# Zhongxu-Wang/ArtSpeech

Hardware: NVIDIA B200
Metric: synthesized_audio_seconds_per_second (higher is better)
Workload: dtype bf16 (vocoder) / f16 (acoustic) operands, f32 accumulate

## Files before the change

### artspeech_b200/csrc/conv_igemm_impl.cuh

```cuda
#pragma once
#include "tc_util.cuh"

namespace asb {

constexpr int CV_THREADS = 320;
constexpr int CV_MAX_TAPS = 32;

struct ConvArgs {
  int B, To, Fo, Cout, CoutP;
  int tT, tF, n_ttiles, n_ftiles;
  int ntaps, kchunks, stages;
  int tap_dt[CV_MAX_TAPS];
  int tap_df[CV_MAX_TAPS];
  uint32_t idesc;
  const float* bias;
  const void* res1; int res1_dtype; long long res1_ld;
  const void* res2; int res2_dtype; long long res2_ld;
  float out_scale;
  void* y_raw; int y_raw_dtype; long long y_raw_ld; int y_raw_vec;
  void* y_act; int y_act_dtype; long long y_act_ld; int y_act_vec;
  int act; float slope;
  const int* lens;
  float* stats;
  int fast, k_res1, k_res2, k_raw, k_act, act_simple;
  float act_slope_eff;
  int halo_rows, pad_lo;
  int epi_tma;
  int halo_baseoff;
  int skip;
  int pad_stages;
};

struct EpiMaps { CUtensorMap r1, raw, act; };
__host__ __device__ constexpr uint32_t epi_cols(int bn) { return bn >= 64 ? 64u : 32u; }
__host__ __device__ constexpr uint32_t epi_warp_bytes(int bn) { return 2u * 32u * epi_cols(bn) * 2u; }
__host__ __device__ constexpr uint32_t epi_bytes(int bn) { return 8u * epi_warp_bytes(bn) + 64u; }


__device__ __forceinline__ bool conv_mtile_dead(const ConvArgs& a, int mt) {
  const int m = mt / a.n_ftiles;
  const int tt = m % a.n_ttiles, b = m / a.n_ttiles;
  if (b >= a.B) return true;
  return tt * a.tT >= __ldg(a.lens + b);
}
__device__ __forceinline__ bool conv_unit_skip(const ConvArgs& a, int unit, int cl) {
  if (!a.skip) return false;
  for (int r = 0; r < cl; ++r)
    if (!conv_mtile_dead(a, unit * cl + r)) return false;
  return true;
}
__device__ __forceinline__ void conv_zero_row(void* base, int dtype, long long off_elems, int ncols) {
  const int es = dtype == AS_F32 ? 4 : 2;
  char* p = reinterpret_cast<char*>(base) + off_elems * es;
  const int nbytes = ncols * es;
  int i = 0;
  if ((reinterpret_cast<uintptr_t>(p) & 15) == 0)
    for (; i + 16 <= nbytes; i += 16) *reinterpret_cast<uint4*>(p + i) = make_uint4(0u, 0u, 0u, 0u);
  for (; i < nbytes; i += es) {
    if (es == 4) *reinterpret_cast<float*>(p + i) = 0.f;
    else *reinterpret_cast<uint16_t*>(p + i) = 0;
  }
}
__device__ __forceinline__ void conv_zero_tile_row(const ConvArgs& a, int mt, int n0, int bn, int m) {
  const int it_ = m / a.tF, if_ = m - it_ * a.tF;
  int u = mt;
  const int ft = u % a.n_ftiles; u /= a.n_ftiles;
  const int tt = u % a.n_ttiles; u /= a.n_ttiles;
  const int b = u, t = tt * a.tT + it_, f = ft * a.tF + if_;
  if (b >= a.B || t >= a.To || f >= a.Fo) return;
  const int ncols = min(bn, a.Cout - n0);
  if (ncols <= 0) return;
  const long long row = ((long long)b * a.To + t) * a.Fo + f;
  if (a.y_raw != nullptr) conv_zero_row(a.y_raw, a.y_raw_dtype, row * a.y_raw_ld + n0, ncols);
  if (a.y_act != nullptr) conv_zero_row(a.y_act, a.y_act_dtype, row * a.y_act_ld + n0, ncols);
}

__device__ __forceinline__ void store16(void* base, int dtype, long long off, const float (&v)[16],
                                        int nvalid, bool vec) {
  if (dtype == AS_F32) {
    float* p = reinterpret_cast<float*>(base) + off;
    if (vec && nvalid == 16) {
      float4* p4 = reinterpret_cast<float4*>(p);
#pragma unroll
// ... 37 lines not shown
    if (vec && nvalid == 16) {
      const uint4* p4 = reinterpret_cast<const uint4*>(p);
#pragma unroll
      for (int h = 0; h < 2; ++h) {
        uint4 t = __ldg(p4 + h);
        uint32_t w[4] = {t.x, t.y, t.z, t.w};
#pragma unroll
        for (int i = 0; i < 4; ++i) {
          v[8 * h + 2 * i] += from16(uint16_t(w[i] & 0xFFFF), dtype);
          v[8 * h + 2 * i + 1] += from16(uint16_t(w[i] >> 16), dtype);
        }
      }
    } else {
#pragma unroll
      for (int i = 0; i < 16; ++i) if (i < nvalid) v[i] += from16(p[i], dtype);
    }
  }
}


template <bool BF16>
__device__ __forceinline__ void add_res_fast(const char* p, int kind, float (&v)[16]) {
  if (kind == 1) {
    const uint4 t0 = __ldg(reinterpret_cast<const uint4*>(p)), t1 = __ldg(reinterpret_cast<const uint4*>(p) + 1);
    unpack_add<BF16>(t0.x, v[0], v[1]); unpack_add<BF16>(t0.y, v[2], v[3]);
    unpack_add<BF16>(t0.z, v[4], v[5]); unpack_add<BF16>(t0.w, v[6], v[7]);
    unpack_add<BF16>(t1.x, v[8], v[9]); unpack_add<BF16>(t1.y, v[10], v[11]);
    unpack_add<BF16>(t1.z, v[12], v[13]); unpack_add<BF16>(t1.w, v[14], v[15]);
  } else {
#pragma unroll
    for (int i = 0; i < 4; ++i) {
      const float4 t = __ldg(reinterpret_cast<const float4*>(p) + i);
      v[4 * i] += t.x; v[4 * i + 1] += t.y; v[4 * i + 2] += t.z; v[4 * i + 3] += t.w;
    }
  }
}
template <bool BF16>
__device__ __forceinline__ void store_fast(char* p, int kind, const float (&v)[16]) {
  if (kind == 1) {
    uint4* q = reinterpret_cast<uint4*>(p);
    q[0] = make_uint4(pack2<BF16>(v[0], v[1]), pack2<BF16>(v[2], v[3]), pack2<BF16>(v[4], v[5]), pack2<BF16>(v[6], v[7]));
    q[1] = make_uint4(pack2<BF16>(v[8], v[9]), pack2<BF16>(v[10], v[11]), pack2<BF16>(v[12], v[13]), pack2<BF16>(v[14], v[15]));
  } else {
    float4* q = reinterpret_cast<float4*>(p);
#pragma unroll
    for (int i = 0; i < 4; ++i) q[i] = make_float4(v[4 * i], v[4 * i + 1], v[4 * i + 2], v[4 * i + 3]);
  }
}

template <int BN, bool BF16>
__device__ __forceinline__ void run_epilogue(const ConvArgs& a, uint32_t tmem_base, uint32_t tfull0,
                                             uint32_t tempty0, int warp, int lane, int m_tiles,
                                             int total_tiles, const float* bias_s, int tile_first = -1,
                                             int tile_step = 0, int cl = 1, int rank = 0, bool remote_tempty = false) {
  if (tile_first < 0) { tile_first = blockIdx.x; tile_step = gridDim.x; }
  constexpr int NPRE = (BN >= 256 ? 128 : (BN < 64 ? BN : 64)) / 8;
  auto tfull_bar = [&](int i) { return tfull0 + 8u * i; };
  auto tempty_bar = [&](int i) { return tempty0 + 8u * i; };
    const int wg = (warp - 2) >> 2;
  const int q = warp & 3;
  const int m = q * 32 + lane;
  const int it_ = m / a.tF, if_ = m - it_ * a.tF;
  int lt_live = 0;
  for (int tile = tile_first; tile < total_tiles; tile += tile_step) {
    if (conv_unit_skip(a, tile % m_tiles, cl)) {
      if (wg == 0) conv_zero_tile_row(a, (tile % m_tiles) * cl + rank, (tile / m_tiles) * BN, BN, m);
      continue;
    }
    const int lt = lt_live++;
    if ((lt & 1) != wg) continue;
    int mt = (tile % m_tiles) * cl + rank;
    const int n0 = (tile / m_tiles) * BN;
    const int ft = mt % a.n_ftiles; mt /= a.n_ftiles;
    const int tt = mt % a.n_ttiles; mt /= a.n_ttiles;
    const int b = mt;
    const int t = tt * a.tT + it_, f = ft * a.tF + if_;
    const bool row_ok = (t < a.To) && (f < a.Fo) && (b < a.B);
    bool masked = false;
    if (a.lens != nullptr && row_ok) masked = t >= __ldg(a.lens + b);
    const long long row = ((long long)b * a.To + t) * a.Fo + f;

    const int ncols = min(BN, a.Cout - n0);
    const bool fast = a.fast != 0;
    const int k_r1 = a.k_res1, k_r2 = a.k_res2, k_raw = a.k_raw, k_act = a.k_act;
    const char* p_r1 = k_r1 ? reinterpret_cast<const char*>(a.res1) + (row * a.res1_ld + n0) * (k_r1 == 1 ? 2 : 4) : nullptr;
    const char* p_r2 = k_r2 ? reinterpret_cast<const char*>(a.res2) + (row * a.res2_ld + n0) * (k_r2 == 1 ? 2 : 4) : nullptr;
    char* p_raw = k_raw ? reinterpret_cast<char*>(a.y_raw) + (row * a.y_raw_ld + n0) * (k_raw == 1 ? 2 : 4) : nullptr;
    char* p_act = k_act ? reinterpret_cast<char*>(a.y_act) + (row * a.y_act_ld + n0) * (k_act == 1 ? 2 : 4) : nullptr;
    const float scale = masked ? 0.f : a.out_scale;
    const float aslope = a.act_slope_eff;
    const float* bias_t = bias_s + n0;
    const bool pre_ok = fast && k_r1 == 1 && row_ok && !masked;
    uint4 pre[NPRE];
    if (pre_ok) {
#pragma unroll
      for (int i = 0; i < NPRE; ++i)
        if (i * 8 + 8 <= ncols) pre[i] = __ldg(reinterpret_cast<const uint4*>(p_r1) + i);
    }

    mbar_wait(tfull_bar(wg), ((uint32_t)lt >> 1) & 1u);
    tc_fence_after();
    const uint32_t tacc = tmem_base + (uint32_t)(wg * BN) + (uint32_t(q * 32) << 16);
#pragma unroll
    for (int cc = 0; cc < BN / 16; ++cc) {
      const int c0 = cc * 16;
      if (c0 >= ncols) break;
      uint32_t r[16];
      tc_ld16(tacc + uint32_t(c0), r);
      tc_wait_ld();
      if (!row_ok) continue;
      const int co = n0 + c0;
      float v[16];
#pragma unroll
      for (int i = 0; i < 16; ++i) v[i] = __uint_as_float(r[i]);
      if (fast && c0 + 16 <= ncols) {
        {
#pragma unroll
// ... 5 lines not shown
        if (pre_ok && 2 * cc + 1 < NPRE) {
          const uint4 t0 = pre[(2 * cc) < NPRE ? 2 * cc : 0], t1 = pre[(2 * cc + 1) < NPRE ? 2 * cc + 1 : 0];
          unpack_add<BF16>(t0.x, v[0], v[1]); unpack_add<BF16>(t0.y, v[2], v[3]);
          unpack_add<BF16>(t0.z, v[4], v[5]); unpack_add<BF16>(t0.w, v[6], v[7]);
          unpack_add<BF16>(t1.x, v[8], v[9]); unpack_add<BF16>(t1.y, v[10], v[11]);
          unpack_add<BF16>(t1.z, v[12], v[13]); unpack_add<BF16>(t1.w, v[14], v[15]);
        } else if (k_r1 && !masked) add_res_fast<BF16>(p_r1 + c0 * (k_r1 == 1 ? 2 : 4), k_r1, v);
        if (k_r2 && !masked) add_res_fast<BF16>(p_r2 + c0 * (k_r2 == 1 ? 2 : 4), k_r2, v);
#pragma unroll
        for (int i = 0; i < 16; ++i) v[i] *= scale;
        if (k_raw) store_fast<BF16>(p_raw + c0 * (k_raw == 1 ? 2 : 4), k_raw, v);
        if (k_act) {
          if (a.act_simple) {
#pragma unroll
            for (int i = 0; i < 16; ++i) v[i] = fmaxf(v[i], v[i] * aslope);
          } else {
#pragma unroll
            for (int i = 0; i < 16; ++i) v[i] = apply_act(v[i], a.act, a.slope);
          }
          store_fast<BF16>(p_act + c0 * (k_act == 1 ? 2 : 4), k_act, v);
        }
      } else {
        const int nvalid = min(16, a.Cout - co);
        if (a.bias != nullptr) {
#pragma unroll
          for (int i = 0; i < 16; ++i) if (i < nvalid) v[i] += __ldg(a.bias + co + i);
        }
        if (a.res1 != nullptr) add_res16(a.res1, a.res1_dtype, row * a.res1_ld + co, v, nvalid, false);
        if (a.res2 != nullptr) add_res16(a.res2, a.res2_dtype, row * a.res2_ld + co, v, nvalid, false);
#pragma unroll
        for (int i = 0; i < 16; ++i) v[i] = masked ? 0.f : v[i] * a.out_scale;
        if (a.y_raw != nullptr) store16(a.y_raw, a.y_raw_dtype, row * a.y_raw_ld + co, v, nvalid, false);
        if (a.y_act != nullptr) {
#pragma unroll
          for (int i = 0; i < 16; ++i) v[i] = apply_act(v[i], a.act, a.slope);
          store16(a.y_act, a.y_act_dtype, row * a.y_act_ld + co, v, nvalid, false);
        }
      }
    }
    tc_fence_before();
    __syncwarp();
    if (lane == 0) {
      if (remote_tempty) asm volatile("mbarrier.arrive.release.cluster.shared::cluster.b64 _, [%0];" ::"r"(tempty_bar(wg)) : "memory");
      else asm volatile("mbarrier.arrive.shared::cta.b64 _, [%0];" ::"r"(tempty_bar(wg)) : "memory");
    }
  }
}

template <int BN, bool BF16, bool F32 = false>
__device__ __forceinline__ void run_epilogue_tma(const ConvArgs& a, const EpiMaps& maps, uint32_t tmem_base,
                                                 uint32_t tfull0, uint32_t tempty0, int warp, int lane, int m_tiles,
                                                 int total_tiles, const float* bias_s, uint32_t epi_base,
                                                 int tile_first = -1, int tile_step = 0, int cl = 1, int rank = 0,
                                                 bool remote_tempty = false) {
  if (tile_first < 0) { tile_first = blockIdx.x; tile_step = gridDim.x; }
  const int ew = warp - 2;
  const int wg = ew >> 2;
  const int q = warp & 3;
  constexpr uint32_t EPC = F32 ? 32u : epi_cols(BN);
  constexpr uint32_t ROWA = F32 ? 128u : EPC * 2u;
  constexpr uint32_t ROWB = EPC * 2u;
  constexpr uint32_t TILEA = 32u * ROWA;
  constexpr int CPG = EPC / 16;
  const uint32_t bufA = epi_base + (uint32_t)ew * epi_warp_bytes(BN);
  const uint32_t bufB = bufA + epi_warp_bytes(BN) / 2u;
  const uint32_t rbar = epi_base + 8u * epi_warp_bytes(BN) + 8u * ew;
  const bool has_r1 = a.k_res1 != 0, has_raw = a.k_raw != 0, has_act = a.k_act != 0;
  const uint32_t rowoffA = (uint32_t)lane * ROWA, rowoffB = (uint32_t)lane * ROWB;
  const uint32_t swA = (ROWA == 128) ? (uint32_t)(lane & 7) : (uint32_t)((lane >> 1) & 3);
  const uint32_t swB = (ROWB == 128) ? (uint32_t)(lane & 7) : (uint32_t)((lane >> 1) & 3);
  uint32_t rphase = 0;
  int lt_live = 0;
  for (int tile = tile_first; tile < total_tiles; tile += tile_step) {
    if (conv_unit_skip(a, tile % m_tiles, cl)) {
      if (wg == 0) conv_zero_tile_row(a, (tile % m_tiles) * cl + rank, (tile / m_tiles) * BN, BN, q * 32 + lane);
      continue;
    }
    const int lt = lt_live++;
    if ((lt & 1) != wg) continue;
    const int mt = (tile % m_tiles) * cl + rank;
    const int n0 = (tile / m_tiles) * BN;
    const int tt = mt % a.n_ttiles, b = mt / a.n_ttiles;
    const int t_base = tt * 128 + q * 32;
    const int t = t_base + lane;
    const bool masked = (a.lens != nullptr) && (b < a.B) && (t < a.To) && (t >= __ldg(a.lens + b));
    const int ncols = min(BN, a.Cout - n0);
    const int ngroups = (ncols + (int)EPC - 1) / (int)EPC;
    const float scale = a.out_scale, aslope = a.act_slope_eff;

    if (has_r1 && lane == 0 && ngroups > 0) {
      bulk_wait_read0();
      mbar_expect_tx(rbar, TILEA);
      tma_load_3d(bufA, &maps.r1, rbar, n0, t_base, b);
    }
    mbar_wait(tfull0 + 8u * wg, ((uint32_t)lt >> 1) & 1u);
    tc_fence_after();
    const uint32_t tacc = tmem_base + (uint32_t)(wg * BN) + (uint32_t(q * 32) << 16);
    for (int g = 0; g < ngroups; ++g) {
      if (has_r1) {
        mbar_wait(rbar, rphase);
        rphase ^= 1u;
      } else {
        if (lane == 0) bulk_wait_read0();
        __syncwarp();
      }
#pragma unroll
      for (int cc = 0; cc < CPG; ++cc) {
        const int c0 = g * (int)EPC + cc * 16;
        if (c0 < ncols) {
          uint32_t r[16];
          tc_ld16(tacc + uint32_t(c0), r);
          tc_wait_ld();
          float v[16];
          const float* bt = bias_s + n0 + c0;
#pragma unroll
          for (int i = 0; i < 4; ++i) {
            const float4 bb = *reinterpret_cast<const float4*>(bt + 4 * i);
            v[4 * i] = __uint_as_float(r[4 * i]) + bb.x; v[4 * i + 1] = __uint_as_float(r[4 * i + 1]) + bb.y;
            v[4 * i + 2] = __uint_as_float(r[4 * i + 2]) + bb.z; v[4 * i + 3] = __uint_as_float(r[4 * i + 3]) + bb.w;
          }
          if constexpr (F32) {
            uint32_t oa[4];
#pragma unroll
            for (int j = 0; j < 4; ++j) oa[j] = bufA + rowoffA + (((uint32_t)(4 * cc + j) ^ swA) << 4);
            if (has_r1) {
#pragma unroll
// ... 37 lines not shown
            }
            const uint32_t b0 = bufB + rowoffB + (((uint32_t)(2 * cc) ^ swB) << 4), b1 = bufB + rowoffB + (((uint32_t)(2 * cc + 1) ^ swB) << 4);
            sts128(b0, make_uint4(pack2<BF16>(v[0], v[1]), pack2<BF16>(v[2], v[3]), pack2<BF16>(v[4], v[5]), pack2<BF16>(v[6], v[7])));
            sts128(b1, make_uint4(pack2<BF16>(v[8], v[9]), pack2<BF16>(v[10], v[11]), pack2<BF16>(v[12], v[13]), pack2<BF16>(v[14], v[15])));
          }
        }
      }
      fence_async_smem();
      __syncwarp();
      if (lane == 0) {
        if (has_raw) tma_store_3d(&maps.raw, bufA, n0 + g * (int)EPC, t_base, b);
        if (has_act) tma_store_3d(&maps.act, bufB, n0 + g * (int)EPC, t_base, b);
        bulk_commit();
        if (has_r1 && g + 1 < ngroups) {
          bulk_wait_read0();
          mbar_expect_tx(rbar, TILEA);
          tma_load_3d(bufA, &maps.r1, rbar, n0 + (g + 1) * (int)EPC, t_base, b);
        }
      }
      __syncwarp();
    }
    tc_fence_before();
    __syncwarp();
    if (lane == 0) {
      if (remote_tempty) asm volatile("mbarrier.arrive.release.cluster.shared::cluster.b64 _, [%0];" ::"r"(tempty0 + 8u * wg) : "memory");
      else asm volatile("mbarrier.arrive.shared::cta.b64 _, [%0];" ::"r"(tempty0 + 8u * wg) : "memory");
    }
  }
  if (lane == 0) bulk_wait_all0();
}

template <int BN, int BK, bool BF16>
__global__ void __launch_bounds__(CV_THREADS, (BN >= 256 ? 1 : 2))
conv_igemm_kernel(const __grid_constant__ CUtensorMap tmA, const __grid_constant__ CUtensorMap tmW,
                  const __grid_constant__ EpiMaps emaps,
                  const __grid_constant__ ConvArgs a) {
  constexpr int A_BYTES = 128 * BK * 2;
  constexpr int W_BYTES = BN * BK * 2;
  constexpr int STAGE_BYTES = A_BYTES + W_BYTES;
  constexpr int TMEM_COLS = (2 * BN) < 32 ? 32 : (2 * BN);

  extern __shared__ unsigned char smem_dyn[];
  const uint32_t smem_base = (smem_u32(smem_dyn) + 1023u) & ~1023u;
  const int S = a.stages;
  const uint32_t bar_base = smem_base + S * STAGE_BYTES;
  auto full_bar = [&](int s) { return bar_base + 8u * s; };
  auto empty_bar = [&](int s) { return bar_base + 8u * (S + s); };
  auto tfull_bar = [&](int i) { return bar_base + 8u * (2 * S + i); };
  auto tempty_bar = [&](int i) { return bar_base + 8u * (2 * S + 2 + i); };
  const uint32_t tmem_slot = bar_base + 8u * (2 * S + 4);
  float* bias_s = reinterpret_cast<float*>(smem_dyn + (bar_base + 8u * (2 * S + 6) - smem_u32(smem_dyn)));
  for (int i = threadIdx.x; i < a.CoutP; i += blockDim.x) bias_s[i] = (a.bias != nullptr && i < a.Cout) ? a.bias[i] : 0.f;
  const uint32_t epi_base = (bar_base + 8u * (2 * S + 6) + (uint32_t)a.CoutP * 4u + 1023u) & ~1023u;

  const int warp = threadIdx.x >> 5;
  const int lane = threadIdx.x & 31;
  const int m_tiles = a.B * a.n_ttiles * a.n_ftiles;
  const int total_tiles = m_tiles * (a.CoutP / BN);
  const int k_iters = a.ntaps * a.kchunks;

  if (threadIdx.x == 0) {
    for (int s = 0; s < S; ++s) { mbar_init(full_bar(s), 1); mbar_init(empty_bar(s), 1); }
    for (int i = 0; i < 2; ++i) { mbar_init(tfull_bar(i), 1); mbar_init(tempty_bar(i), 4); }
    if (a.epi_tma) for (int i = 0; i < 8; ++i) mbar_init(epi_base + 8u * epi_warp_bytes(BN) + 8u * i, 1);
    asm volatile("fence.mbarrier_init.release.cluster;" ::: "memory");
  }
  if (warp == 0 && lane == 0) {
    asm volatile("prefetch.tensormap [%0];" ::"l"(&tmA) : "memory");
    asm volatile("prefetch.tensormap [%0];" ::"l"(&tmW) : "memory");
  }
  if (warp == 1) {
    asm volatile("tcgen05.alloc.cta_group::1.sync.aligned.shared::cta.b32 [%0], %1;" ::"r"(tmem_slot),
                 "n"(TMEM_COLS)
                 : "memory");
    asm volatile("tcgen05.relinquish_alloc_permit.cta_group::1.sync.aligned;" ::: "memory");
  }
  tc_fence_before();
  __syncthreads();
  tc_fence_after();
  pdl_wait();
  uint32_t tmem_base;
  asm volatile("ld.shared.b32 %0, [%1];" : "=r"(tmem_base) : "r"(tmem_slot) : "memory");

  if (warp == 0) {
    if (lane == 0) {
      int it = 0;
      for (int tile = blockIdx.x; tile < total_tiles; tile += gridDim.x) {
        if (conv_unit_skip(a, tile % m_tiles, 1)) continue;
        int mt = tile % m_tiles;
        const int n0 = (tile / m_tiles) * BN;
        const int ft = mt % a.n_ftiles; mt /= a.n_ftiles;
        const int tt = mt % a.n_ttiles; mt /= a.n_ttiles;
        const int b = mt, t0 = tt * a.tT, f0 = ft * a.tF;
        for (int kit = 0; kit < k_iters; ++kit, ++it) {
          const int s = it % S;
          const uint32_t ph = (it / S) & 1;
          mbar_wait(empty_bar(s), ph ^ 1u);
          mbar_expect_tx(full_bar(s), STAGE_BYTES);
          const int tap = kit / a.kchunks, kc = kit - tap * a.kchunks;
          const uint32_t sa = smem_base + s * STAGE_BYTES;
          tma_load_4d(sa, &tmA, full_bar(s), kc * BK, f0 + a.tap_df[tap], t0 + a.tap_dt[tap], b);
          tma_load_2d(sa + A_BYTES, &tmW, full_bar(s), kc * BK, tap * a.CoutP + n0);
        }
      }
    }
  } else if (warp == 1) {
    if (elect_one()) {
      int it = 0, lt = 0;
      for (int tile = blockIdx.x; tile < total_tiles; tile += gridDim.x) {
        if (conv_unit_skip(a, tile % m_tiles, 1)) continue;
        const int acc = lt & 1;
        mbar_wait(tempty_bar(acc), (((uint32_t)lt >> 1) & 1u) ^ 1u);
        tc_fence_after();
        const uint32_t tacc = tmem_base + (uint32_t)(acc * BN);
        for (int kit = 0; kit < k_iters; ++kit, ++it) {
          const int s = it % S;
          const uint32_t ph = (it / S) & 1;
          mbar_wait(full_bar(s), ph);
          tc_fence_after();
          const uint32_t sa = smem_base + s * STAGE_BYTES;
          const uint64_t da = make_smem_desc<BK>(sa);
          const uint64_t db = make_smem_desc<BK>(sa + A_BYTES);
#pragma unroll
          for (int k = 0; k < BK / 16; ++k) {
            tc_mma_f16(tacc, da + uint64_t(2 * k), db + uint64_t(2 * k), a.idesc, (kit | k) != 0 ? 1u : 0u);
          }
          tc_commit(empty_bar(s));
        }
        tc_commit(tfull_bar(acc));
        ++lt;
      }
    }
  } else {
    if (a.epi_tma == 2) {
      if constexpr (BN >= 128)
        run_epilogue_tma<BN, BF16, true>(a, emaps, tmem_base, tfull_bar(0), tempty_bar(0), warp, lane, m_tiles, total_tiles, bias_s, epi_base);
    } else if (a.epi_tma)
      run_epilogue_tma<BN, BF16>(a, emaps, tmem_base, tfull_bar(0), tempty_bar(0), warp, lane, m_tiles, total_tiles, bias_s, epi_base);
    else
      run_epilogue<BN, BF16>(a, tmem_base, tfull_bar(0), tempty_bar(0), warp, lane, m_tiles, total_tiles, bias_s);
  }

  tc_fence_before();
  __syncthreads();
  if (warp == 1) {
    tc_fence_after();
    asm volatile("tcgen05.dealloc.cta_group::1.sync.aligned.b32 %0, %1;" ::"r"(tmem_base),
                 "n"(TMEM_COLS)
                 : "memory");
  }
}


template <int BK, bool BF16>
__global__ void __cluster_dims__(2, 1, 1) __launch_bounds__(CV_THREADS, 1)
conv_igemm_2cta_kernel(const __grid_constant__ CUtensorMap tmA, const __grid_constant__ CUtensorMap tmWh,
                       const __grid_constant__ EpiMaps emaps, const __grid_constant__ ConvArgs a) {
  constexpr int BN = 256;
  constexpr int A_BYTES = 128 * BK * 2;
  constexpr int WH_BYTES = (BN / 2) * BK * 2;
  constexpr int STAGE_BYTES = A_BYTES + WH_BYTES;
  constexpr int TMEM_COLS = 512;

  extern __shared__ unsigned char smem_dyn[];
  const uint32_t smem_base = ((smem_u32(smem_dyn) + 1023u) & ~1023u) + (uint32_t)a.pad_stages * STAGE_BYTES;
  const int S = a.stages;
  const uint32_t bar_base = smem_base + S * STAGE_BYTES;
  auto full_bar = [&](int s) { return bar_base + 8u * s; };
  auto empty_bar = [&](int s) { return bar_base + 8u * (S + s); };
  auto tfull_bar = [&](int i) { return bar_base + 8u * (2 * S + i); };
  auto tempty_bar = [&](int i) { return bar_base + 8u * (2 * S + 2 + i); };
  const uint32_t tmem_slot = bar_base + 8u * (2 * S + 4);
  float* bias_s = reinterpret_cast<float*>(smem_dyn + (bar_base + 8u * (2 * S + 6) - smem_u32(smem_dyn)));
  for (int i = threadIdx.x; i < a.CoutP; i += blockDim.x) bias_s[i] = (a.bias != nullptr && i < a.Cout) ? a.bias[i] : 0.f;
  const uint32_t epi_base = (bar_base + 8u * (2 * S + 6) + (uint32_t)a.CoutP * 4u + 1023u) & ~1023u;

  const int warp = threadIdx.x >> 5;
  const int lane = threadIdx.x & 31;
  const uint32_t rank = cluster_ctarank();
  const bool leader = rank == 0;
  const int m_tiles = a.B * a.n_ttiles * a.n_ftiles;
  const int m_pairs = (m_tiles + 1) / 2;
  const int total_super = m_pairs * (a.CoutP / BN);
  const int cid = blockIdx.x >> 1, n_clusters = gridDim.x >> 1;
  const int k_iters = a.ntaps * a.kchunks;

  if (threadIdx.x == 0) {
    for (int s = 0; s < S; ++s) { mbar_init(full_bar(s), 1); mbar_init(empty_bar(s), 1); }
    for (int i = 0; i < 2; ++i) { mbar_init(tfull_bar(i), 1); mbar_init(tempty_bar(i), 8); }
    if (a.epi_tma) for (int i = 0; i < 8; ++i) mbar_init(epi_base + 8u * epi_warp_bytes(BN) + 8u * i, 1);
    asm volatile("fence.mbarrier_init.release.cluster;" ::: "memory");
  }
  if (warp == 0 && lane == 0) {
    asm volatile("prefetch.tensormap [%0];" ::"l"(&tmA) : "memory");
    asm volatile("prefetch.tensormap [%0];" ::"l"(&tmWh) : "memory");
  }
  if (warp == 1) {
    asm volatile("tcgen05.alloc.cta_group::2.sync.aligned.shared::cta.b32 [%0], %1;" ::"r"(tmem_slot), "n"(TMEM_COLS) : "memory");
    asm volatile("tcgen05.relinquish_alloc_permit.cta_group::2.sync.aligned;" ::: "memory");
  }
  tc_fence_before();
  cluster_sync();
  tc_fence_after();
  pdl_wait();
  uint32_t tmem_base;
  asm volatile("ld.shared.b32 %0, [%1];" : "=r"(tmem_base) : "r"(tmem_slot) : "memory");

  if (warp == 0) {
    if (lane == 0) {
      int it = 0;
      for (int st = cid; st < total_super; st += n_clusters) {
        if (conv_unit_skip(a, st % m_pairs, 2)) continue;
        int mt = (st % m_pairs) * 2 + (int)rank;
        const int n0 = (st / m_pairs) * BN;
        const int ft = mt % a.n_ftiles; mt /= a.n_ftiles;
        const int tt = mt % a.n_ttiles; mt /= a.n_ttiles;
        const int b = mt, t0 = tt * a.tT, f0 = ft * a.tF;
        for (int kit = 0; kit < k_iters; ++kit, ++it) {
          const int s = it % S;
          const uint32_t ph = (it / S) & 1;
          mbar_wait(empty_bar(s), ph ^ 1u);
          if (leader) mbar_expect_tx(full_bar(s), 2u * STAGE_BYTES);
          const uint32_t fb = mapa_u32(full_bar(s), 0);
          const int tap = kit / a.kchunks, kc = kit - tap * a.kchunks;
          const uint32_t sa = smem_base + s * STAGE_BYTES;
          tma2_load_4d(sa, &tmA, fb, kc * BK, f0 + a.tap_df[tap], t0 + a.tap_dt[tap], b);
          tma2_load_2d(sa + A_BYTES, &tmWh, fb, kc * BK, tap * a.CoutP + n0 + (int)rank * (BN / 2));
        }
      }
    }
  } else if (warp == 1) {
    if (leader && elect_one()) {
      int it = 0, lt = 0;
      for (int st = cid; st < total_super; st += n_clusters) {
        if (conv_unit_skip(a, st % m_pairs, 2)) continue;
        const int acc = lt & 1;
        mbar_wait(tempty_bar(acc), (((uint32_t)lt >> 1) & 1u) ^ 1u);
        tc_fence_after();
        const uint32_t tacc = tmem_base + (uint32_t)(acc * BN);
        for (int kit = 0; kit < k_iters; ++kit, ++it) {
          const int s = it % S;
          const uint32_t ph = (it / S) & 1;
          mbar_wait(full_bar(s), ph);
          tc_fence_after();
          const uint32_t sa = smem_base + s * STAGE_BYTES;
          const uint64_t da = make_smem_desc<BK>(sa);
          const uint64_t db = make_smem_desc<BK>(sa + A_BYTES);
#pragma unroll
          for (int k = 0; k < BK / 16; ++k)
            tc2_mma_f16(tacc, da + uint64_t(2 * k), db + uint64_t(2 * k), a.idesc, (kit | k) != 0 ? 1u : 0u);
          tc2_commit(empty_bar(s));
        }
        tc2_commit(tfull_bar(acc));
        ++lt;
      }
    }
    __syncwarp();
  } else {
    const uint32_t tempty_leader = mapa_u32(tempty_bar(0), 0);
    if (a.epi_tma == 2)
      run_epilogue_tma<BN, BF16, true>(a, emaps, tmem_base, tfull_bar(0), tempty_leader, warp, lane, m_pairs, total_super, bias_s,
                                       epi_base, cid, n_clusters, 2, (int)rank, true);
    else if (a.epi_tma)
      run_epilogue_tma<BN, BF16>(a, emaps, tmem_base, tfull_bar(0), tempty_leader, warp, lane, m_pairs, total_super, bias_s, epi_base,
                                 cid, n_clusters, 2, (int)rank, true);
    else
      run_epilogue<BN, BF16>(a, tmem_base, tfull_bar(0), tempty_leader, warp, lane, m_pairs, total_super, bias_s,
                             cid, n_clusters, 2, (int)rank, true);
  }

  tc_fence_before();
  cluster_sync();
  if (warp == 1) {
    tc_fence_after();
    asm volatile("tcgen05.dealloc.cta_group::2.sync.aligned.b32 %0, %1;" ::"r"(tmem_base), "n"(TMEM_COLS) : "memory");
  }
}

__device__ __forceinline__ uint64_t make_desc_noswz(uint32_t saddr, uint32_t lbo_bytes) {
  return uint64_t((saddr >> 4) & 0x3FFF) | (uint64_t((lbo_bytes >> 4) & 0x3FFF) << 16) |
         (uint64_t(128 >> 4) << 32) | (uint64_t(1) << 46);
}

template <int BN, bool BF16>
__global__ void __launch_bounds__(CV_THREADS, 2)
conv_halo_kernel(const __grid_constant__ CUtensorMap tmA, const __grid_constant__ CUtensorMap tmW,
                  const __grid_constant__ EpiMaps emaps,
                 const __grid_constant__ ConvArgs a) {
  constexpr int TMEM_COLS = (2 * BN) < 32 ? 32 : (2 * BN);
  extern __shared__ unsigned char smem_dyn[];
  const uint32_t smem_base = (smem_u32(smem_dyn) + 127u) & ~127u;
  const int S = a.stages;
  const int KC = a.kchunks;
  const int HRP = a.halo_rows;
  const uint32_t a_bytes = (uint32_t)KC * HRP * 16;
  const uint32_t w_tap_bytes = (uint32_t)KC * BN * 16;
  const uint32_t w_base = smem_base + S * a_bytes;
  const uint32_t bar_base = (w_base + a.ntaps * w_tap_bytes + 7u) & ~7u;
  auto full_bar = [&](int s) { return bar_base + 8u * s; };
  auto empty_bar = [&](int s) { return bar_base + 8u * (S + s); };
  auto tfull_bar = [&](int i) { return bar_base + 8u * (2 * S + i); };
  auto tempty_bar = [&](int i) { return bar_base + 8u * (2 * S + 2 + i); };
  const uint32_t w_bar = bar_base + 8u * (2 * S + 4);
  const uint32_t tmem_slot = bar_base + 8u * (2 * S + 5);
  float* bias_s = reinterpret_cast<float*>(smem_dyn + (bar_base + 8u * (2 * S + 6) - smem_u32(smem_dyn)));
  for (int i = threadIdx.x; i < a.CoutP; i += blockDim.x) bias_s[i] = (a.bias != nullptr && i < a.Cout) ? a.bias[i] : 0.f;
  const uint32_t epi_base = (bar_base + 8u * (2 * S + 6) + (uint32_t)a.CoutP * 4u + 1023u) & ~1023u;

  const int warp = threadIdx.x >> 5;
  const int lane = threadIdx.x & 31;
  const int m_tiles = a.B * a.n_ttiles;
  const int total_tiles = m_tiles;

  if (threadIdx.x == 0) {
    for (int s = 0; s < S; ++s) { mbar_init(full_bar(s), 1); mbar_init(empty_bar(s), 1); }
    for (int i = 0; i < 2; ++i) { mbar_init(tfull_bar(i), 1); mbar_init(tempty_bar(i), 4); }
    mbar_init(w_bar, 1);
    if (a.epi_tma) for (int i = 0; i < 8; ++i) mbar_init(epi_base + 8u * epi_warp_bytes(BN) + 8u * i, 1);
    asm volatile("fence.mbarrier_init.release.cluster;" ::: "memory");
  }
  if (warp == 0 && lane == 0) {
// ... 172 lines not shown
            for (int k = 0; k < BKC / 16; ++k) {
              tc_mma_f16(tacc, da + uint64_t(2 * k), db + uint64_t(2 * k), a.idesc, first);
              first = 1u;
            }
          }
        }
        tc_commit(empty_bar(s));
        tc_commit(tfull_bar(acc));
      }
    }
  } else {
    if (a.epi_tma)
      run_epilogue_tma<BN, BF16>(a, emaps, tmem_base, tfull_bar(0), tempty_bar(0), warp, lane, m_tiles, total_tiles, bias_s, epi_base);
    else
      run_epilogue<BN, BF16>(a, tmem_base, tfull_bar(0), tempty_bar(0), warp, lane, m_tiles, total_tiles, bias_s);
  }

  tc_fence_before();
  __syncthreads();
  if (warp == 1) {
    tc_fence_after();
    asm volatile("tcgen05.dealloc.cta_group::1.sync.aligned.b32 %0, %1;" ::"r"(tmem_base),
                 "n"(TMEM_COLS)
                 : "memory");
  }
}


inline int pick_tile_n(int Cout) {
  if (Cout <= 16) return 16;
  if (Cout <= 32) return 32;
  if (Cout <= 64) return 64;
  if (Cout <= 128) return 128;
  if (Cout % 256 == 0) return 256;
  if (Cout % 128 == 0) return 128;
  int p256 = (Cout + 255) / 256 * 256, p128 = (Cout + 127) / 128 * 128;
  return p128 < p256 ? 128 : 256;
}


template <int BN, int BK, bool BF16>
int launch_conv(const CUtensorMap& tmA, const CUtensorMap& tmW, const EpiMaps& em, ConvArgs& a,
                       int total_tiles, cudaStream_t st) {
  constexpr int STAGE_BYTES = 128 * BK * 2 + BN * BK * 2;
  const int ctas_per_sm = (BN >= 256 || a.epi_tma) ? 1 : 2;
  const int budget = a.epi_tma ? (222 * 1024 - (int)epi_bytes(BN) - 2048 - a.CoutP * 4)
                               : ((BN >= 256 ? 208 : 104) * 1024 - a.CoutP * 4);
  int stages = budget / STAGE_BYTES;
  if (stages > 10) stages = 10;
  if (stages < 2) stages = 2;
  a.stages = stages;
  static const bool no_skip = getenv("ASB_CONV_NO_SKIP") != nullptr;
  a.skip = (a.lens != nullptr && !no_skip) ? 1 : 0;
  const size_t smem = (size_t)stages * STAGE_BYTES + 8 * (2 * stages + 6) + (size_t)a.CoutP * 4 + 1024 + 16 +
                      (a.epi_tma ? epi_bytes(BN) + 1024 : 0);
  ASB_SMEM_OPT_IN(227 * 1024, conv_igemm_kernel<BN, BK, BF16>);
  int grid = num_sms() * ctas_per_sm;
  if (grid > total_tiles) grid = total_tiles;
  ASB_CUDA(launch_k(conv_igemm_kernel<BN, BK, BF16>, grid, CV_THREADS, smem, st, tmA, tmW, em, a));
  ASB_CUDA(cudaGetLastError());
  return AS_OK;
}

template <int BK, bool BF16>
int launch_conv_2cta(const CUtensorMap& tmA, const CUtensorMap& tmWh, const EpiMaps& em, ConvArgs& a, cudaStream_t st) {
  constexpr int BN = 256;
  constexpr int STAGE_BYTES = 128 * BK * 2 + (BN / 2) * BK * 2;
  const int budget = a.epi_tma ? (222 * 1024 - (int)epi_bytes(BN) - 2048 - a.CoutP * 4) : (208 * 1024 - a.CoutP * 4);
  int stages = budget / STAGE_BYTES;
  static const int max_stages = getenv("ASB_2CTA_STAGES") ? atoi(getenv("ASB_2CTA_STAGES")) : 4;
  if (stages > max_stages) stages = max_stages;
  if (stages < 2) stages = 2;
  a.stages = stages;
  static const int pad = getenv("ASB_2CTA_PAD") ? atoi(getenv("ASB_2CTA_PAD")) : 0;
  a.pad_stages = (stages + pad) * STAGE_BYTES <= budget ? pad : 0;
  a.idesc = (a.idesc & ~(0x1Fu << 24)) | (uint32_t(256 >> 4) << 24);
  static const bool no_skip = getenv("ASB_CONV_NO_SKIP") != nullptr;
  a.skip = (a.lens != nullptr && !no_skip) ? 1 : 0;
  const size_t smem = (size_t)(stages + a.pad_stages) * STAGE_BYTES + 8 * (2 * stages + 6) + (size_t)a.CoutP * 4 + 1024 + 16 +
                      (a.epi_tma ? epi_bytes(BN) + 1024 : 0);
  ASB_SMEM_OPT_IN(227 * 1024, conv_igemm_2cta_kernel<BK, BF16>);
  const int m_tiles = a.B * a.n_ttiles * a.n_ftiles;
  const int total_super = ((m_tiles + 1) / 2) * (a.CoutP / BN);
  int clusters = num_sms() / 2;
  if (clusters > total_super) clusters = total_super;
  ASB_CUDA(launch_k(conv_igemm_2cta_kernel<BK, BF16>, 2 * clusters, CV_THREADS, smem, st, tmA, tmWh, em, a));
  return AS_OK;
}

template <int BN, bool BF16>
int launch_halo(const as_conv_params* p, ConvArgs& a, const EpiMaps& em, EncodeTiledFn enc, cudaStream_t st) {
  const int KC = p->Cin / 8;
  int lo = 0, hi = 0;
  for (int j = 0; j < p->ntaps; ++j) { lo = p->tap_dt[j] < lo ? p->tap_dt[j] : lo; hi = p->tap_dt[j] > hi ? p->tap_dt[j] : hi; }
  const int HRP = (128 + hi - lo + 7) / 8 * 8;
  a.kchunks = KC; a.halo_rows = HRP; a.pad_lo = -lo; a.skip = 0;
  a.tT = 128; a.tF = 1; a.n_ttiles = (p->To + 127) / 128; a.n_ftiles = 1;
  const size_t a_bytes = (size_t)KC * HRP * 16, w_bytes = (size_t)p->ntaps * KC * BN * 16;
  int stages = 4;
  while (stages > 2 && stages * a_bytes + w_bytes > 190 * 1024) --stages;
  a.stages = stages;
  const size_t epi = a.epi_tma ? epi_bytes(BN) + 1024 : 0;
  while (stages > 2 && stages * a_bytes + w_bytes + epi > 208 * 1024) --stages;
  a.stages = stages;
  const size_t smem = stages * a_bytes + w_bytes + 8 * (2 * stages + 6) + (size_t)a.CoutP * 4 + 256 + 16 + epi;
  const CUtensorMapDataType dt = BF16 ? CU_TENSOR_MAP_DATA_TYPE_BFLOAT16 : CU_TENSOR_MAP_DATA_TYPE_FLOAT16;
  CUtensorMap tmA, tmW;
  {
    cuuint64_t dims[4] = {8, (cuuint64_t)p->T, (cuuint64_t)KC, (cuuint64_t)p->B};
    cuuint64_t strides[3] = {(cuuint64_t)p->x_ld * 2, 16, (cuuint64_t)p->x_ld * 2 * p->T};
    cuuint32_t box[4] = {8, (cuuint32_t)HRP, (cuuint32_t)KC, 1};
    cuuint32_t es[4] = {1, 1, 1, 1};
    CUresult r = enc(&tmA, dt, 4, const_cast<void*>(p->x), dims, strides, box, es, CU_TENSOR_MAP_INTERLEAVE_NONE,
                     CU_TENSOR_MAP_SWIZZLE_NONE, CU_TENSOR_MAP_L2_PROMOTION_L2_128B, CU_TENSOR_MAP_FLOAT_OOB_FILL_NONE);
    ASB_REQUIRE(r == CUDA_SUCCESS, AS_ERR_CUDA, "cuTensorMapEncodeTiled(halo A) failed: %d", (int)r);
  }
  {
    cuuint64_t dims[4] = {8, (cuuint64_t)p->ntaps * p->CoutP, (cuuint64_t)KC, 1};
    cuuint64_t strides[3] = {(cuuint64_t)p->CinP * 2, 16, (cuuint64_t)p->CinP * 2 * p->ntaps * p->CoutP};
    cuuint32_t box[4] = {8, (cuuint32_t)BN, (cuuint32_t)KC, 1};
    cuuint32_t es[4] = {1, 1, 1, 1};
    CUresult r = enc(&tmW, dt, 4, const_cast<void*>(p->w), dims, strides, box, es, CU_TENSOR_MAP_INTERLEAVE_NONE,
                     CU_TENSOR_MAP_SWIZZLE_NONE, CU_TENSOR_MAP_L2_PROMOTION_L2_256B, CU_TENSOR_MAP_FLOAT_OOB_FILL_NONE);
    ASB_REQUIRE(r == CUDA_SUCCESS, AS_ERR_CUDA, "cuTensorMapEncodeTiled(halo W) failed: %d", (int)r);
  }
  ASB_SMEM_OPT_IN(227 * 1024, conv_halo_kernel<BN, BF16>);
  const int total_tiles = p->B * a.n_ttiles;
  int per_sm = (int)((220 * 1024) / (smem + 1024));
  if (per_sm > 2) per_sm = 2;
  if (per_sm < 1) per_sm = 1;
  int grid = num_sms() * per_sm;
  if (grid > total_tiles) grid = total_tiles;
  ASB_CUDA(launch_k(conv_halo_kernel<BN, BF16>, grid, CV_THREADS, smem, st, tmA, tmW, em, a));
  ASB_CUDA(cudaGetLastError());
  return AS_OK;
}

// ... 54 lines not shown
```

### artspeech_b200/csrc/tc_util.cuh

```cuda
#pragma once
#include <cuda.h>
#include <stdlib.h>
#include <string.h>

#include "common.cuh"

namespace asb {

__device__ __forceinline__ void mbar_init(uint32_t bar, uint32_t count) {
  asm volatile("mbarrier.init.shared::cta.b64 [%0], %1;" ::"r"(bar), "r"(count));
}
__device__ __forceinline__ void mbar_expect_tx(uint32_t bar, uint32_t bytes) {
  asm volatile("mbarrier.arrive.expect_tx.shared::cta.b64 _, [%0], %1;" ::"r"(bar), "r"(bytes)
               : "memory");
}
__device__ __forceinline__ void mbar_wait(uint32_t bar, uint32_t parity) {
  asm volatile(
      "{\n"
      ".reg .pred p;\n"
      "WAIT_%=:\n"
      "mbarrier.try_wait.parity.shared::cta.b64 p, [%0], %1;\n"
      "@p bra DONE_%=;\n"
      "bra WAIT_%=;\n"
      "DONE_%=:\n"
// ... 84 lines not shown

__device__ __forceinline__ uint32_t cluster_ctarank() {
  uint32_t r;
  asm volatile("mov.u32 %0, %%cluster_ctarank;" : "=r"(r));
  return r;
}
__device__ __forceinline__ uint32_t mapa_u32(uint32_t addr, uint32_t rank) {
  uint32_t r;
  asm volatile("mapa.shared::cluster.u32 %0, %1, %2;" : "=r"(r) : "r"(addr), "r"(rank));
  return r;
}
__device__ __forceinline__ void cluster_sync() {
  asm volatile("barrier.cluster.arrive.release.aligned;\n\tbarrier.cluster.wait.acquire.aligned;" ::: "memory");
}
__device__ __forceinline__ void tma2_load_4d(uint32_t dst, const CUtensorMap* map, uint32_t bar_cluster, int c0, int c1, int c2, int c3) {
  asm volatile(
      "cp.async.bulk.tensor.4d.cta_group::2.shared::cluster.global.tile.mbarrier::complete_tx::bytes "
      "[%0], [%1, {%3, %4, %5, %6}], [%2];" ::"r"(dst), "l"(map), "r"(bar_cluster), "r"(c0), "r"(c1), "r"(c2), "r"(c3)
      : "memory");
}
__device__ __forceinline__ void tma2_load_2d(uint32_t dst, const CUtensorMap* map, uint32_t bar_cluster, int c0, int c1) {
  asm volatile(
      "cp.async.bulk.tensor.2d.cta_group::2.shared::cluster.global.tile.mbarrier::complete_tx::bytes "
      "[%0], [%1, {%3, %4}], [%2];" ::"r"(dst), "l"(map), "r"(bar_cluster), "r"(c0), "r"(c1)
      : "memory");
}
__device__ __forceinline__ void tc2_mma_f16(uint32_t tmem_d, uint64_t da, uint64_t db, uint32_t idesc, uint32_t accumulate) {
  asm volatile(
      "{\n"
      ".reg .pred p;\n"
      "setp.ne.b32 p, %4, 0;\n"
      "tcgen05.mma.cta_group::2.kind::f16 [%0], %1, %2, %3, p;\n"
      "}\n" ::"r"(tmem_d),
      "l"(da), "l"(db), "r"(idesc), "r"(accumulate)
      : "memory");
}
__device__ __forceinline__ void tc2_commit(uint32_t bar) {
  asm volatile("tcgen05.commit.cta_group::2.mbarrier::arrive::one.shared::cluster.multicast::cluster.b64 [%0], %1;" ::"r"(bar),
               "h"((uint16_t)3)
               : "memory");
}

__device__ __forceinline__ void tma2_load_3d(uint32_t dst, const CUtensorMap* map, uint32_t bar_cluster, int c0, int c1, int c2) {
  asm volatile(
      "cp.async.bulk.tensor.3d.cta_group::2.shared::cluster.global.tile.mbarrier::complete_tx::bytes "
      "[%0], [%1, {%3, %4, %5}], [%2];" ::"r"(dst), "l"(map), "r"(bar_cluster), "r"(c0), "r"(c1), "r"(c2)
      : "memory");
}
__device__ __forceinline__ void mbar_arrive_cluster(uint32_t bar_cluster) {
  asm volatile("mbarrier.arrive.release.cluster.shared::cluster.b64 _, [%0];" ::"r"(bar_cluster) : "memory");
}
__device__ __forceinline__ void mbar_arrive_cluster_relaxed(uint32_t bar_cluster) {
  asm volatile("mbarrier.arrive.relaxed.cluster.shared::cluster.b64 _, [%0];" ::"r"(bar_cluster) : "memory");
}

template <int BK>
__device__ __forceinline__ uint64_t make_smem_desc(uint32_t saddr) {
  constexpr uint64_t sbo = (BK == 64 ? 1024 : 512) >> 4;
  constexpr uint64_t layout = (BK == 64) ? 2 : 4;
  return uint64_t((saddr >> 4) & 0x3FFF) | (uint64_t(1) << 16) | (sbo << 32) | (uint64_t(1) << 46) |
         (layout << 61);
}

template <bool BF16>
__device__ __forceinline__ uint32_t pack2(float a, float b) {
  if (BF16) { __nv_bfloat162 t = __floats2bfloat162_rn(a, b); return *reinterpret_cast<uint32_t*>(&t); }
  __half2 t = __floats2half2_rn(a, b);
  return *reinterpret_cast<uint32_t*>(&t);
}
template <bool BF16>
__device__ __forceinline__ void unpack_add(uint32_t u, float& a, float& b) {
  if (BF16) { a += __uint_as_float(u << 16); b += __uint_as_float(u & 0xFFFF0000u); return; }
  const float2 f = __half22float2(*reinterpret_cast<const __half2*>(&u));
  a += f.x; b += f.y;
}

typedef CUresult (*EncodeTiledFn)(CUtensorMap*, CUtensorMapDataType, cuuint32_t, void*,
                                  const cuuint64_t*, const cuuint64_t*, const cuuint32_t*,
                                  const cuuint32_t*, CUtensorMapInterleave, CUtensorMapSwizzle,
                                  CUtensorMapL2promotion, CUtensorMapFloatOOBfill);

inline EncodeTiledFn get_encode_fn() {
  static EncodeTiledFn fn = nullptr;
  if (fn) return fn;
  void* p = nullptr;
  cudaDriverEntryPointQueryResult qres;
  cudaError_t e = cudaGetDriverEntryPoint("cuTensorMapEncodeTiled", &p, cudaEnableDefault, &qres);
  if (e != cudaSuccess || qres != cudaDriverEntryPointSuccess || p == nullptr) {
    set_error("cuTensorMapEncodeTiled unavailable (err %d)", (int)e);
    return nullptr;
  }
  fn = reinterpret_cast<EncodeTiledFn>(p);
  return fn;
}

extern int g_sm_limit;

inline int num_sms_device() {
  static std::atomic<int> cache[64];
  int dev = 0;
  cudaGetDevice(&dev);
  std::atomic<int>& slot = cache[dev & 63];
  int n = slot.load(std::memory_order_relaxed);
  if (n == 0) {
    cudaDeviceGetAttribute(&n, cudaDevAttrMultiProcessorCount, dev);
    if (n <= 0) n = 148;
    slot.store(n, std::memory_order_relaxed);
  }
  return n;
}

inline int num_sms() {
  const int n = num_sms_device();
  return g_sm_limit > 0 ? std::max(2, std::min(n, g_sm_limit) & ~1) : n;
}

}
```

Before: 10620.

## Use cluster launch control for dynamic tile scheduling in conv implicit-GEMM kernels

Replaces the static persistent grid-stride tile loop with dynamic tile scheduling built on Blackwell cluster launch control (try_cancel/query_cancel). The grid is launched with one CTA per tile, and running CTAs cancel not-yet-launched CTAs to claim their tiles. A small shared-memory ring with mbarriers hands claimed tile ids to the TMA issuer, MMA, and epilogue warps, including the peer CTA in 2-CTA clusters. The goal is better load balance when tiles are skipped (length masking) or uneven, at the cost of extra barrier traffic and more complex synchronization.

New measurement: 10860, median of 6. 1.02x the previous value.

```diff
diff --git a/artspeech_b200/csrc/conv_igemm_impl.cuh b/artspeech_b200/csrc/conv_igemm_impl.cuh
--- a/artspeech_b200/csrc/conv_igemm_impl.cuh
+++ b/artspeech_b200/csrc/conv_igemm_impl.cuh
@@ -29,6 +29,7 @@
   int halo_baseoff;
   int skip;
   int pad_stages;
+  int dyn;
 };
 
 struct EpiMaps { CUtensorMap r1, raw, act; };
@@ -172,8 +173,10 @@
 __device__ __forceinline__ void run_epilogue(const ConvArgs& a, uint32_t tmem_base, uint32_t tfull0,
                                              uint32_t tempty0, int warp, int lane, int m_tiles,
                                              int total_tiles, const float* bias_s, int tile_first = -1,
-                                             int tile_step = 0, int cl = 1, int rank = 0, bool remote_tempty = false) {
+                                             int tile_step = 0, int cl = 1, int rank = 0, bool remote_tempty = false,
+                                             uint32_t ts_ring = 0) {
   if (tile_first < 0) { tile_first = blockIdx.x; tile_step = gridDim.x; }
+  TileWalk tw = ts_walk(tile_step, total_tiles, ts_ring);
   constexpr int NPRE = (BN >= 256 ? 128 : (BN < 64 ? BN : 64)) / 8;
   auto tfull_bar = [&](int i) { return tfull0 + 8u * i; };
   auto tempty_bar = [&](int i) { return tempty0 + 8u * i; };
@@ -182,7 +185,8 @@
   const int m = q * 32 + lane;
   const int it_ = m / a.tF, if_ = m - it_ * a.tF;
   int lt_live = 0;
-  for (int tile = tile_first; tile < total_tiles; tile += tile_step) {
+  auto next = [&](int t) { return cl == 2 ? ts_next<TS_WARP_READER, 1>(tw, t, rank != 0) : ts_next<TS_WARP_READER>(tw, t); };
+  for (int tile = ts_first<TS_WARP_READER>(tw, tile_first); tile >= 0; tile = next(tile)) {
     if (conv_unit_skip(a, tile % m_tiles, cl)) {
       if (wg == 0) conv_zero_tile_row(a, (tile % m_tiles) * cl + rank, (tile / m_tiles) * BN, BN, m);
       continue;
@@ -294,8 +298,9 @@
                                                  uint32_t tfull0, uint32_t tempty0, int warp, int lane, int m_tiles,
                                                  int total_tiles, const float* bias_s, uint32_t epi_base,
                                                  int tile_first = -1, int tile_step = 0, int cl = 1, int rank = 0,
-                                                 bool remote_tempty = false) {
+                                                 bool remote_tempty = false, uint32_t ts_ring = 0) {
   if (tile_first < 0) { tile_first = blockIdx.x; tile_step = gridDim.x; }
+  TileWalk tw = ts_walk(tile_step, total_tiles, ts_ring);
   const int ew = warp - 2;
   const int wg = ew >> 2;
   const int q = warp & 3;
@@ -313,7 +318,8 @@
   const uint32_t swB = (ROWB == 128) ? (uint32_t)(lane & 7) : (uint32_t)((lane >> 1) & 3);
   uint32_t rphase = 0;
   int lt_live = 0;
-  for (int tile = tile_first; tile < total_tiles; tile += tile_step) {
+  auto next = [&](int t) { return cl == 2 ? ts_next<TS_WARP_READER, 1>(tw, t, rank != 0) : ts_next<TS_WARP_READER>(tw, t); };
+  for (int tile = ts_first<TS_WARP_READER>(tw, tile_first); tile >= 0; tile = next(tile)) {
     if (conv_unit_skip(a, tile % m_tiles, cl)) {
       if (wg == 0) conv_zero_tile_row(a, (tile % m_tiles) * cl + rank, (tile / m_tiles) * BN, BN, q * 32 + lane);
       continue;
@@ -457,6 +463,7 @@
   float* bias_s = reinterpret_cast<float*>(smem_dyn + (bar_base + 8u * (2 * S + 6) - smem_u32(smem_dyn)));
   for (int i = threadIdx.x; i < a.CoutP; i += blockDim.x) bias_s[i] = (a.bias != nullptr && i < a.Cout) ? a.bias[i] : 0.f;
   const uint32_t epi_base = (bar_base + 8u * (2 * S + 6) + (uint32_t)a.CoutP * 4u + 1023u) & ~1023u;
+  const uint32_t ts_ring = a.dyn ? epi_base + (a.epi_tma ? epi_bytes(BN) : 0u) : 0u;
 
   const int warp = threadIdx.x >> 5;
   const int lane = threadIdx.x & 31;
@@ -468,6 +475,7 @@
     for (int s = 0; s < S; ++s) { mbar_init(full_bar(s), 1); mbar_init(empty_bar(s), 1); }
     for (int i = 0; i < 2; ++i) { mbar_init(tfull_bar(i), 1); mbar_init(tempty_bar(i), 4); }
     if (a.epi_tma) for (int i = 0; i < 8; ++i) mbar_init(epi_base + 8u * epi_warp_bytes(BN) + 8u * i, 1);
+    if (ts_ring) ts_init(ts_ring, 10);
     asm volatile("fence.mbarrier_init.release.cluster;" ::: "memory");
   }
   if (warp == 0 && lane == 0) {
@@ -490,7 +498,8 @@
   if (warp == 0) {
     if (lane == 0) {
       int it = 0;
-      for (int tile = blockIdx.x; tile < total_tiles; tile += gridDim.x) {
+      TileWalk tw = ts_walk(gridDim.x, total_tiles, ts_ring);
+      for (int tile = ts_first<TS_ISSUER>(tw, blockIdx.x); tile >= 0; tile = ts_next<TS_ISSUER>(tw, tile)) {
         if (conv_unit_skip(a, tile % m_tiles, 1)) continue;
         int mt = tile % m_tiles;
         const int n0 = (tile / m_tiles) * BN;
@@ -512,7 +521,8 @@
   } else if (warp == 1) {
     if (elect_one()) {
       int it = 0, lt = 0;
-      for (int tile = blockIdx.x; tile < total_tiles; tile += gridDim.x) {
+      TileWalk tw = ts_walk(gridDim.x, total_tiles, ts_ring);
+      for (int tile = ts_first<TS_READER>(tw, blockIdx.x); tile >= 0; tile = ts_next<TS_READER>(tw, tile)) {
         if (conv_unit_skip(a, tile % m_tiles, 1)) continue;
         const int acc = lt & 1;
         mbar_wait(tempty_bar(acc), (((uint32_t)lt >> 1) & 1u) ^ 1u);
@@ -539,11 +549,14 @@
   } else {
     if (a.epi_tma == 2) {
       if constexpr (BN >= 128)
-        run_epilogue_tma<BN, BF16, true>(a, emaps, tmem_base, tfull_bar(0), tempty_bar(0), warp, lane, m_tiles, total_tiles, bias_s, epi_base);
+        run_epilogue_tma<BN, BF16, true>(a, emaps, tmem_base, tfull_bar(0), tempty_bar(0), warp, lane, m_tiles, total_tiles, bias_s,
+                                         epi_base, -1, 0, 1, 0, false, ts_ring);
     } else if (a.epi_tma)
-      run_epilogue_tma<BN, BF16>(a, emaps, tmem_base, tfull_bar(0), tempty_bar(0), warp, lane, m_tiles, total_tiles, bias_s, epi_base);
+      run_epilogue_tma<BN, BF16>(a, emaps, tmem_base, tfull_bar(0), tempty_bar(0), warp, lane, m_tiles, total_tiles, bias_s, epi_base,
+                                 -1, 0, 1, 0, false, ts_ring);
     else
-      run_epilogue<BN, BF16>(a, tmem_base, tfull_bar(0), tempty_bar(0), warp, lane, m_tiles, total_tiles, bias_s);
+      run_epilogue<BN, BF16>(a, tmem_base, tfull_bar(0), tempty_bar(0), warp, lane, m_tiles, total_tiles, bias_s, -1, 0, 1, 0, false,
+                             ts_ring);
   }
 
   tc_fence_before();
@@ -579,6 +592,7 @@
   float* bias_s = reinterpret_cast<float*>(smem_dyn + (bar_base + 8u * (2 * S + 6) - smem_u32(smem_dyn)));
   for (int i = threadIdx.x; i < a.CoutP; i += blockDim.x) bias_s[i] = (a.bias != nullptr && i < a.Cout) ? a.bias[i] : 0.f;
   const uint32_t epi_base = (bar_base + 8u * (2 * S + 6) + (uint32_t)a.CoutP * 4u + 1023u) & ~1023u;
+  const uint32_t ts_ring = a.dyn ? epi_base + (a.epi_tma ? epi_bytes(BN) : 0u) : 0u;
 
   const int warp = threadIdx.x >> 5;
   const int lane = threadIdx.x & 31;
@@ -594,6 +608,7 @@
     for (int s = 0; s < S; ++s) { mbar_init(full_bar(s), 1); mbar_init(empty_bar(s), 1); }
     for (int i = 0; i < 2; ++i) { mbar_init(tfull_bar(i), 1); mbar_init(tempty_bar(i), 8); }
     if (a.epi_tma) for (int i = 0; i < 8; ++i) mbar_init(epi_base + 8u * epi_warp_bytes(BN) + 8u * i, 1);
+    if (ts_ring) ts_init(ts_ring, 19);
     asm volatile("fence.mbarrier_init.release.cluster;" ::: "memory");
   }
   if (warp == 0 && lane == 0) {
@@ -614,7 +629,10 @@
   if (warp == 0) {
     if (lane == 0) {
       int it = 0;
-      for (int st = cid; st < total_super; st += n_clusters) {
+      TileWalk tw = ts_walk(n_clusters, total_super, ts_ring);
+      auto first = [&](int t) { return leader ? ts_first<TS_ISSUER, 1>(tw, t) : ts_first<TS_PEER_ISSUER, 1>(tw, t); };
+      auto next = [&](int t) { return leader ? ts_next<TS_ISSUER, 1>(tw, t) : ts_next<TS_PEER_ISSUER, 1>(tw, t, true); };
+      for (int st = first(cid); st >= 0; st = next(st)) {
         if (conv_unit_skip(a, st % m_pairs, 2)) continue;
         int mt = (st % m_pairs) * 2 + (int)rank;
         const int n0 = (st / m_pairs) * BN;
@@ -637,7 +655,8 @@
   } else if (warp == 1) {
     if (leader && elect_one()) {
       int it = 0, lt = 0;
-      for (int st = cid; st < total_super; st += n_clusters) {
+      TileWalk tw = ts_walk(n_clusters, total_super, ts_ring);
+      for (int st = ts_first<TS_READER, 1>(tw, cid); st >= 0; st = ts_next<TS_READER, 1>(tw, st)) {
         if (conv_unit_skip(a, st % m_pairs, 2)) continue;
         const int acc = lt & 1;
         mbar_wait(tempty_bar(acc), (((uint32_t)lt >> 1) & 1u) ^ 1u);
@@ -665,13 +684,13 @@
     const uint32_t tempty_leader = mapa_u32(tempty_bar(0), 0);
     if (a.epi_tma == 2)
       run_epilogue_tma<BN, BF16, true>(a, emaps, tmem_base, tfull_bar(0), tempty_leader, warp, lane, m_pairs, total_super, bias_s,
-                                       epi_base, cid, n_clusters, 2, (int)rank, true);
+                                       epi_base, cid, n_clusters, 2, (int)rank, true, ts_ring);
     else if (a.epi_tma)
       run_epilogue_tma<BN, BF16>(a, emaps, tmem_base, tfull_bar(0), tempty_leader, warp, lane, m_pairs, total_super, bias_s, epi_base,
-                                 cid, n_clusters, 2, (int)rank, true);
+                                 cid, n_clusters, 2, (int)rank, true, ts_ring);
     else
       run_epilogue<BN, BF16>(a, tmem_base, tfull_bar(0), tempty_leader, warp, lane, m_pairs, total_super, bias_s,
-                             cid, n_clusters, 2, (int)rank, true);
+                             cid, n_clusters, 2, (int)rank, true, ts_ring);
   }
 
   tc_fence_before();
@@ -950,10 +969,11 @@
   a.stages = stages;
   static const bool no_skip = getenv("ASB_CONV_NO_SKIP") != nullptr;
   a.skip = (a.lens != nullptr && !no_skip) ? 1 : 0;
+  a.dyn = dynamic_tiles() ? 1 : 0;
   const size_t smem = (size_t)stages * STAGE_BYTES + 8 * (2 * stages + 6) + (size_t)a.CoutP * 4 + 1024 + 16 +
-                      (a.epi_tma ? epi_bytes(BN) + 1024 : 0);
+                      (a.epi_tma ? epi_bytes(BN) + 1024 : 0) + TS_BYTES;
   ASB_SMEM_OPT_IN(227 * 1024, conv_igemm_kernel<BN, BK, BF16>);
-  int grid = num_sms() * ctas_per_sm;
+  int grid = a.dyn ? total_tiles : num_sms() * ctas_per_sm;
   if (grid > total_tiles) grid = total_tiles;
   ASB_CUDA(launch_k(conv_igemm_kernel<BN, BK, BF16>, grid, CV_THREADS, smem, st, tmA, tmW, em, a));
   ASB_CUDA(cudaGetLastError());
@@ -975,12 +995,13 @@
   a.idesc = (a.idesc & ~(0x1Fu << 24)) | (uint32_t(256 >> 4) << 24);
   static const bool no_skip = getenv("ASB_CONV_NO_SKIP") != nullptr;
   a.skip = (a.lens != nullptr && !no_skip) ? 1 : 0;
+  a.dyn = dynamic_tiles() ? 1 : 0;
   const size_t smem = (size_t)(stages + a.pad_stages) * STAGE_BYTES + 8 * (2 * stages + 6) + (size_t)a.CoutP * 4 + 1024 + 16 +
-                      (a.epi_tma ? epi_bytes(BN) + 1024 : 0);
+                      (a.epi_tma ? epi_bytes(BN) + 1024 : 0) + TS_BYTES;
   ASB_SMEM_OPT_IN(227 * 1024, conv_igemm_2cta_kernel<BK, BF16>);
   const int m_tiles = a.B * a.n_ttiles * a.n_ftiles;
   const int total_super = ((m_tiles + 1) / 2) * (a.CoutP / BN);
-  int clusters = num_sms() / 2;
+  int clusters = a.dyn ? total_super : num_sms() / 2;
   if (clusters > total_super) clusters = total_super;
   ASB_CUDA(launch_k(conv_igemm_2cta_kernel<BK, BF16>, 2 * clusters, CV_THREADS, smem, st, tmA, tmWh, em, a));
   return AS_OK;
diff --git a/artspeech_b200/csrc/tc_util.cuh b/artspeech_b200/csrc/tc_util.cuh
--- a/artspeech_b200/csrc/tc_util.cuh
+++ b/artspeech_b200/csrc/tc_util.cuh
@@ -160,6 +160,78 @@
 }
 __device__ __forceinline__ void mbar_arrive_cluster_relaxed(uint32_t bar_cluster) {
   asm volatile("mbarrier.arrive.relaxed.cluster.shared::cluster.b64 _, [%0];" ::"r"(bar_cluster) : "memory");
+}
+
+constexpr int TS_DEPTH = 4;
+constexpr uint32_t TS_BYTES = TS_DEPTH * 16u + 2u * TS_DEPTH * 8u;
+__device__ __forceinline__ uint32_t ts_resp(uint32_t ring, uint32_t i) { return ring + 16u * i; }
+__device__ __forceinline__ uint32_t ts_full(uint32_t ring, uint32_t i) { return ring + 16u * TS_DEPTH + 8u * i; }
+__device__ __forceinline__ uint32_t ts_empty(uint32_t ring, uint32_t i) { return ring + 24u * TS_DEPTH + 8u * i; }
+struct TileWalk {
+  int step, total;
+  uint32_t ring;
+  uint32_t n;
+};
+enum { TS_READER = 0, TS_WARP_READER = 1, TS_ISSUER = 2, TS_PEER_ISSUER = 3 };
+
+__device__ __forceinline__ void ts_init(uint32_t ring, uint32_t readers) {
+  for (uint32_t i = 0; i < TS_DEPTH; ++i) { mbar_init(ts_full(ring, i), 1); mbar_init(ts_empty(ring, i), readers); }
+}
+__device__ __forceinline__ TileWalk ts_walk(int step, int total, uint32_t ring) {
+  TileWalk w;
+  w.step = step; w.total = total; w.ring = ring; w.n = 0;
+  return w;
+}
+template <int ROLE, int SHIFT>
+__device__ __forceinline__ void ts_request(const TileWalk& w) {
+  const uint32_t i = w.n % TS_DEPTH;
+  if (ROLE == TS_ISSUER) {
+    mbar_wait(ts_empty(w.ring, i), ((w.n / TS_DEPTH) & 1u) ^ 1u);
+    mbar_expect_tx(ts_full(w.ring, i), 16u);
+    if (SHIFT)
+      asm volatile("clusterlaunchcontrol.try_cancel.async.shared::cta.mbarrier::complete_tx::bytes.multicast::cluster::all.b128 [%0], [%1];"
+                   ::"r"(ts_resp(w.ring, i)), "r"(ts_full(w.ring, i)) : "memory");
+    else
+      asm volatile("clusterlaunchcontrol.try_cancel.async.shared::cta.mbarrier::complete_tx::bytes.b128 [%0], [%1];"
+                   ::"r"(ts_resp(w.ring, i)), "r"(ts_full(w.ring, i)) : "memory");
+  } else if (ROLE == TS_PEER_ISSUER) {
+    mbar_expect_tx(ts_full(w.ring, i), 16u);
+  }
+}
+template <int ROLE, int SHIFT = 0>
+__device__ __forceinline__ int ts_first(const TileWalk& w, int first) {
+  if (first >= w.total) return -1;
+  if (w.ring) ts_request<ROLE, SHIFT>(w);
+  return first;
+}
+template <int ROLE, int SHIFT = 0>
+__device__ __forceinline__ int ts_next(TileWalk& w, int unit, bool remote = false) {
+  if (!w.ring) {
+    unit += w.step;
+    return unit < w.total ? unit : -1;
+  }
+  const uint32_t i = w.n % TS_DEPTH;
+  mbar_wait(ts_full(w.ring, i), (w.n / TS_DEPTH) & 1u);
+  uint32_t ok, x = 0;
+  asm volatile(
+      "{\n"
+      ".reg .pred p;\n"
+      ".reg .b128 v;\n"
+      "ld.shared.b128 v, [%2];\n"
+      "clusterlaunchcontrol.query_cancel.is_canceled.pred.b128 p, v;\n"
+      "selp.u32 %0, 1, 0, p;\n"
+      "@p clusterlaunchcontrol.query_cancel.get_first_ctaid::x.b32.b128 %1, v;\n"
+      "}\n"
+      : "=r"(ok), "+r"(x) : "r"(ts_resp(w.ring, i)) : "memory");
+  unit = ok ? (int)(x >> SHIFT) : -1;
+  if (ROLE == TS_WARP_READER) __syncwarp();
+  if (ROLE != TS_WARP_READER || (threadIdx.x & 31) == 0) {
+    if (remote) mbar_arrive_cluster_relaxed(mapa_u32(ts_empty(w.ring, i), 0));
+    else asm volatile("mbarrier.arrive.shared::cta.b64 _, [%0];" ::"r"(ts_empty(w.ring, i)) : "memory");
+  }
+  ++w.n;
+  if (unit >= 0) ts_request<ROLE, SHIFT>(w);
+  return unit;
 }
 
 template <int BK>
@@ -223,4 +295,9 @@
   return g_sm_limit > 0 ? std::max(2, std::min(n, g_sm_limit) & ~1) : n;
 }
 
-}
+inline bool dynamic_tiles() {
+  static const bool off = getenv("ASB_STATIC_TILES") != nullptr && atoi(getenv("ASB_STATIC_TILES")) != 0;
+  return !off && g_sm_limit <= 0;
+}
+
+}
```
